# smdogroup/eigd

Measured on AMD Instinct MI355X. Metric: adjoint_mode_derivatives_per_sec, higher is better.
Workload: dtype f64

## Files before the change

eigd_amd/_ffi.py:

```python

import ctypes as C
import os

import numpy as np

_HERE = os.path.dirname(os.path.abspath(__file__))
LIB_PATH = os.environ.get("EIGD_LIB") or os.path.join(_HERE, "lib", "libeigd_hip.so")

EIGD_E_INVALID, EIGD_E_HIP, EIGD_E_NOTSPD, EIGD_E_INTERNAL = -1, -2, -3, -4


class EigdHipError(RuntimeError):
    """HIP runtime / device failure inside libeigd_hip.so."""


class NotPositiveDefiniteError(np.linalg.LinAlgError):
    """The shifted matrix handed to SpLuOperator is not positive definite."""


_lib = None

c_int, c_i64, c_dbl, c_sz, c_vp = C.c_int, C.c_int64, C.c_double, C.c_size_t, C.c_void_p
P = C.POINTER

_SIGNATURES = {
    "eigd_version": [],
    "eigd_device_count": [P(c_int)],
    "eigd_ctx_create": [c_int, P(c_vp)],
    "eigd_ctx_fork": [c_vp, P(c_vp)],
    "eigd_ctx_destroy": [c_vp],
    "eigd_ctx_make_current": [c_vp],
    "eigd_sync": [c_vp],
    "eigd_malloc": [c_vp, c_sz, P(c_vp)],
    "eigd_free": [c_vp, c_vp],
    "eigd_memset": [c_vp, c_vp, c_int, c_sz],
    "eigd_h2d": [c_vp, c_vp, c_vp, c_sz],
    "eigd_d2h": [c_vp, c_vp, c_vp, c_sz],
    "eigd_d2d": [c_vp, c_vp, c_vp, c_sz],
    "eigd_host_alloc": [c_sz, P(c_vp)],
    "eigd_host_free": [c_vp],
    "eigd_host_register": [c_vp, c_sz],
    "eigd_host_unregister": [c_vp],
    "eigd_mem_info": [c_vp, P(c_sz), P(c_sz)],
    "eigd_timer_start": [c_vp],
    "eigd_timer_stop_ms": [c_vp, P(c_dbl)],
    "eigd_csr_upload": [c_vp, c_int, c_i64, c_vp, c_vp, c_vp, P(c_vp)],
    "eigd_csr_upload_rect": [c_vp, c_int, c_int, c_i64, c_vp, c_vp, c_vp, P(c_vp)],
    "eigd_csr_update_values": [c_vp, c_vp],
    "eigd_csr_transpose_pattern": [c_int, c_int, c_vp, c_vp, c_vp, c_vp, c_vp],
    "eigd_csr_transpose": [c_vp, P(c_vp)],
    "eigd_csr_transpose_refresh": [c_vp, c_vp],
    "eigd_mat_free": [c_vp],
    "eigd_spmm": [c_vp, c_vp, c_int, c_vp, c_int, c_int, c_dbl, c_dbl],
    "eigd_spmm_on": [c_vp, c_vp, c_vp, c_int, c_vp, c_int, c_int, c_dbl, c_dbl],
    "eigd_ccsr_upload": [c_vp, c_int, c_i64, c_vp, c_vp, c_vp, P(c_vp)],
    "eigd_ccsr_update_values_dev": [c_vp, c_vp],
    "eigd_ccsr_conjugate_transpose": [c_vp, P(c_vp)],
    "eigd_ccsr_conjugate_transpose_refresh": [c_vp, c_vp],
    "eigd_ccsr_spmm_on": [c_vp, c_vp, c_vp, c_int, c_vp, c_int, c_int, c_dbl, c_dbl],
    "eigd_expand_values": [c_vp, c_i64, c_i64, c_vp, c_vp, c_vp],
    "eigd_symbolic_create": [c_int, c_vp, c_vp, c_int, c_int, P(c_vp)],
    "eigd_symbolic_create_geom": [c_int, c_vp, c_vp, c_int, c_int, c_int, c_vp, P(c_vp)],
    "eigd_symbolic_free": [c_vp],
    "eigd_symbolic_sizes": [c_vp, c_vp, c_int],
    "eigd_symbolic_sweep_plan": [c_vp, c_int, c_int, c_int, c_vp, c_vp, c_int, P(c_int)],
    "eigd_symbolic_get_i32": [c_vp, C.c_char_p, c_vp, c_i64],
    "eigd_symbolic_get_i64": [c_vp, C.c_char_p, c_vp, c_i64],
    "eigd_factor_create": [c_vp, c_vp, c_vp, P(c_vp)],
    "eigd_factor_create_lu": [c_vp, c_vp, c_vp, P(c_vp)],
    "eigd_factor_refactor": [c_vp, c_vp],
# ... 113 lines not shown
```

eigd_amd/csrc/sparse.hip:

```cpp
#include <algorithm>
#include <cstdint>
#include <vector>

#include "common.h"

struct eigd_mat {
  eigd_ctx* ctx = nullptr;
  int n = 0;
  int ncols = 0;
  int64_t nnz = 0;
  int32_t* indptr = nullptr;
  int32_t* indices = nullptr;
  double* data = nullptr;
  int32_t* rowblocks = nullptr;
  int nblocks = 0;
  int ntiles = 0, umax = 0;
  int tnz_cap = 0;
  int32_t* tile_ptr = nullptr;
  int32_t* ucols = nullptr;
  uint16_t* lidx = nullptr;
  int32_t* tperm = nullptr;
  double* cdata = nullptr;
};

namespace eigd {

constexpr int kTileRows = 32;
constexpr int kTileLds = 40 * 1024;
constexpr int kTileNnz = 1024;
constexpr int kNnzTile = 2048;
constexpr int kMaxRowsTile = 256;


__device__ __forceinline__ int xcd_remap(int b, int nblocks_padded) {
  const int per = nblocks_padded >> 3;
  return (b & 7) * per + (b >> 3);
}

__global__ __launch_bounds__(kThreads) void spmv_stream_kernel(const int32_t* __restrict__ rowblocks, int nblocks,
                                                              int nblocks_padded,
                                                              const int32_t* __restrict__ indptr,
                                                              const int32_t* __restrict__ indices,
                                                              const double* __restrict__ vals,
                                                              const double* __restrict__ x, double* __restrict__ y,
                                                              double alpha, double beta) {
  __shared__ double prod[kNnzTile];
  __shared__ double red[kThreads];
  const int b = xcd_remap(blockIdx.x, nblocks_padded);
  if (b >= nblocks) return;
  const int tid = threadIdx.x;
// ... 62 lines not shown
  const int r = blockIdx.x * RP + threadIdx.x / KP;
  if (r >= n || c >= k) return;
  const int a = indptr[r], z = indptr[r + 1];
  double s = 0.0;
  int e = a;
  for (; e + 8 <= z; e += 8) {
    int col[8];
    double v[8], x[8];
#pragma unroll
    for (int q = 0; q < 8; ++q) {
      col[q] = indices[e + q];
      v[q] = vals[e + q];
    }
#pragma unroll
    for (int q = 0; q < 8; ++q) x[q] = X[static_cast<int64_t>(col[q]) * ldx + c];
#pragma unroll
    for (int q = 0; q < 8; ++q) s = __dadd_rn(s, __dmul_rn(v[q], x[q]));
  }
  for (; e < z; ++e) s = __dadd_rn(s, __dmul_rn(vals[e], X[static_cast<int64_t>(indices[e]) * ldx + c]));
  double* yp = Y + static_cast<int64_t>(r) * ldy + c;
  *yp = (beta == 0.0) ? alpha * s : alpha * s + beta * (*yp);
}

template <int KP, int LANES = 8>
struct SpmmTile {
  static constexpr int CPL = (KP >= LANES) ? KP / LANES : 1;
  static constexpr int LPR = KP / CPL;
  static constexpr int LD = (CPL >= 2) ? KP + 4 : KP + 1;
};

template <int KP, int LANES, bool DOTS = false>
__global__ __launch_bounds__(kThreads) void spmm_tiled_kernel(int n, int k, int ntiles, int tiles_per_xcd,
                                                             const int32_t* __restrict__ tile_ptr,
                                                             const int32_t* __restrict__ ucols,
                                                             const int32_t* __restrict__ indptr,
                                                             const uint16_t* __restrict__ lidx,
                                                             const double* __restrict__ vals,
                                                             const double* __restrict__ X, int ldx,
                                                             double* __restrict__ Y, int ldy, double alpha, double beta,
                                                             int umax, int tnz_cap,
                                                             const double* __restrict__ R = nullptr, int ldr = 0,
                                                             double* __restrict__ dots = nullptr) {
  extern __shared__ __align__(16) double Xs[];
  constexpr int RP = kThreads / KP;
  constexpr int CPL = SpmmTile<KP, LANES>::CPL, LPR = SpmmTile<KP, LANES>::LPR, LD = SpmmTile<KP, LANES>::LD;
  constexpr int RPP = kThreads / LPR;
  constexpr int NR = (kTileRows + RPP - 1) / RPP;
  double* const Vs = Xs + static_cast<size_t>(umax) * LD;
  uint16_t* const Ls = reinterpret_cast<uint16_t*>(Vs + tnz_cap);
  const int tile = (blockIdx.x & 7) * tiles_per_xcd + (blockIdx.x >> 3);
  if (tile >= ntiles) return;
  const int c = threadIdx.x % KP, rr = threadIdx.x / KP;
  const int pl = threadIdx.x % LPR, prow = threadIdx.x / LPR;
  const int u0 = tile_ptr[tile], nu = tile_ptr[tile + 1] - u0;
  const int rend = min(n, (tile + 1) * kTileRows);
  const int e0 = indptr[tile * kTileRows], tnz = indptr[rend] - e0;
  const bool staged = tnz <= tnz_cap;
  constexpr int NQ = kTileNnz / kThreads;
  int ra[NR], rz[NR];
#pragma unroll
  for (int i = 0; i < NR; ++i) {
    const int r = tile * kTileRows + prow + i * RPP;
    ra[i] = (r < rend) ? indptr[r] - e0 : 0;
    rz[i] = (r < rend) ? indptr[r + 1] - e0 : 0;
  }
  double sv[NQ];
  uint16_t sl[NQ];
#pragma unroll
  for (int q = 0; q < NQ; ++q) {
    const int e = threadIdx.x + q * kThreads;
    const bool ok = staged && e < tnz;
    sv[q] = ok ? vals[e0 + e] : 0.0;
    sl[q] = ok ? lidx[e0 + e] : uint16_t(0);
  }
  [[maybe_unused]] double xo[CPL], ro[CPL];
  if constexpr (DOTS) {
    const int r = tile * kTileRows + prow;
#pragma unroll
    for (int t = 0; t < CPL; ++t) {
      const bool ok = r < rend && CPL * pl + t < k;
      xo[t] = ok ? X[static_cast<int64_t>(r) * ldx + CPL * pl + t] : 0.0;
      ro[t] = ok ? R[static_cast<int64_t>(r) * ldr + CPL * pl + t] : 0.0;
    }
  }
  constexpr int SU = 16;
  for (int j0 = 0; j0 < nu; j0 += SU * RP) {
    int col[SU];
    double x[SU];
#pragma unroll
    for (int q = 0; q < SU; ++q) {
      const int j = j0 + q * RP + rr;
      col[q] = (j < nu) ? ucols[u0 + j] : -1;
    }
#pragma unroll
    for (int q = 0; q < SU; ++q) x[q] = (col[q] >= 0 && c < k) ? X[static_cast<int64_t>(col[q]) * ldx + c] : 0.0;
#pragma unroll
    for (int q = 0; q < SU; ++q) {
      const int j = j0 + q * RP + rr;
      if (j < nu) Xs[j * LD + c] = x[q];
    }
  }
  if (staged) {
#pragma unroll
// ... 40 lines not shown
#pragma unroll
        for (int w = 0; w < kThreads / 64; ++w) v += dred[(w * 2 + q) * KP + c2];
        dots[static_cast<int64_t>(tile) * 2 * k + threadIdx.x] = v;
      }
    }
  };
  auto store_row = [&](int r, const double (&s)[CPL]) {
    double* yp = Y + static_cast<int64_t>(r) * ldy + cb;
#pragma unroll
    for (int t = 0; t < CPL; ++t)
      if (cb + t < k) {
        const double yv = (beta == 0.0) ? alpha * s[t] : alpha * s[t] + beta * yp[t];
        yp[t] = yv;
        if constexpr (DOTS) {
          dzr[t] += xo[t] * ro[t];
          dzy[t] += xo[t] * yv;
        }
      }
  };
  const bool active = cb < k;
  if (active && staged) {
#pragma unroll
    for (int i = 0; i < NR; ++i) {
      const int r = tile * kTileRows + prow + i * RPP;
      if (r >= rend) break;
      const int a = ra[i], z = rz[i];
      double s[CPL];
#pragma unroll
      for (int t = 0; t < CPL; ++t) s[t] = 0.0;
      int e = a;
      for (; e + 8 <= z; e += 8) {
        int li[8];
        double v[8], x[8][CPL];
#pragma unroll
        for (int q = 0; q < 8; ++q) {
          li[q] = Ls[e + q];
          v[q] = Vs[e + q];
        }
#pragma unroll
        for (int q = 0; q < 8; ++q) {
          const double* xp = Xs + li[q] * LD + cb;
          if constexpr (CPL >= 2) {
            const double2* xp2 = reinterpret_cast<const double2*>(xp);
#pragma unroll
            for (int t = 0; t < CPL / 2; ++t) {
              const double2 w = xp2[t];
              x[q][2 * t] = w.x;
              x[q][2 * t + 1] = w.y;
            }
          } else {
            x[q][0] = xp[0];
          }
        }
#pragma unroll
        for (int q = 0; q < 8; ++q)
#pragma unroll
          for (int t = 0; t < CPL; ++t) s[t] = __dadd_rn(s[t], __dmul_rn(v[q], x[q][t]));
      }
      for (; e < z; ++e) {
        const double v = Vs[e];
        const double* xp = Xs + Ls[e] * LD + cb;
#pragma unroll
        for (int t = 0; t < CPL; ++t) s[t] = __dadd_rn(s[t], __dmul_rn(v, xp[t]));
      }
      store_row(r, s);
    }
  } else if (active) {
  for (int r = tile * kTileRows + prow; r < rend; r += RPP) {
    const int a = indptr[r], z = indptr[r + 1];
    double s[CPL];
#pragma unroll
    for (int t = 0; t < CPL; ++t) s[t] = 0.0;
    for (int e = a; e < z; ++e) {
      const double v = vals[e];
      const double* xp = Xs + lidx[e] * LD + cb;
#pragma unroll
      for (int t = 0; t < CPL; ++t) s[t] = __dadd_rn(s[t], __dmul_rn(v, xp[t]));
    }
    store_row(r, s);
  }
  }
  finish_dots();
}

__global__ __launch_bounds__(kThreads) void tile_dots_reduce_kernel(const double* __restrict__ dots, int ntiles, int nout,
                                                                   double* __restrict__ out) {
  __shared__ double red[kThreads];
  const int per = kThreads / nout;
  const int o = threadIdx.x % nout, sub = threadIdx.x / nout;
  double v = 0.0;
  if (sub < per)
// ... 88 lines not shown
        si = __dadd_rn(si, pi[q]);
      }
      store(r, sr, si);
    }
  } else {
    double sr = 0.0, si = 0.0;
    for (int ea = e0; ea < e1; ea += kNnzTile) {
      const int ez = min(e1, ea + kNnzTile);
      stage(ea, ez);
      __syncthreads();
      if (tid == 0)
        for (int q = 0; q < ez - ea; ++q) {
          sr = __dadd_rn(sr, pr[q]);
          si = __dadd_rn(si, pi[q]);
        }
      __syncthreads();
    }
    if (tid == 0) store(r0, sr, si);
  }
}

template <bool STAGED>
__global__ __launch_bounds__(kThreads) void cspmm_tiled_kernel(int n, int kb, int kp_log2, int ntiles, int tiles_per_xcd,
                                                              const int32_t* __restrict__ tile_ptr,
                                                              const int32_t* __restrict__ ucols,
                                                              const int32_t* __restrict__ indptr,
                                                              const int32_t* __restrict__ indices,
                                                              const uint16_t* __restrict__ lidx,
                                                              const cdbl2* __restrict__ vals,
                                                              const double* __restrict__ X, int ldx, int imx,
                                                              double* __restrict__ Y, int ldy, int imy, double alpha,
                                                              double beta) {
  extern __shared__ __align__(16) double Xs[];
  const int tile = (blockIdx.x & 7) * tiles_per_xcd + (blockIdx.x >> 3);
  if (tile >= ntiles) return;
  const int kp = 1 << kp_log2;
  const int c = threadIdx.x & (kp - 1), rr = threadIdx.x >> kp_log2;
  const int rpp = kThreads >> kp_log2;
  const int ld = 2 * kp + 1;
  const int rbeg = tile * kTileRows, rend = min(n, rbeg + kTileRows);
  if constexpr (STAGED) {
    const int u0 = tile_ptr[tile], nu = tile_ptr[tile + 1] - u0;
    constexpr int SU = 8;
    for (int j0 = 0; j0 < nu; j0 += SU * rpp) {
      int col[SU];
      double xr[SU], xi[SU];
#pragma unroll
      for (int q = 0; q < SU; ++q) {
        const int j = j0 + q * rpp + rr;
        col[q] = (j < nu) ? ucols[u0 + j] : -1;
      }
#pragma unroll
      for (int q = 0; q < SU; ++q) {
        const bool ok = col[q] >= 0 && c < kb;
        const double* xp = X + static_cast<int64_t>(ok ? col[q] : 0) * ldx + (ok ? c : 0);
        xr[q] = ok ? xp[0] : 0.0;
        xi[q] = ok ? xp[imx] : 0.0;
      }
#pragma unroll
      for (int q = 0; q < SU; ++q) {
        const int j = j0 + q * rpp + rr;
        if (j < nu) {
          Xs[j * ld + c] = xr[q];
          Xs[j * ld + kp + c] = xi[q];
        }
      }
    }
    __syncthreads();
  }
  if (c >= kb) return;
  for (int r = rbeg + rr; r < rend; r += rpp) {
    const int a = indptr[r], z = indptr[r + 1];
    CAcc s;
    int e = a;
    for (; e + 4 <= z; e += 4) {
      cdbl2 v[4];
      double xr[4], xi[4];
#pragma unroll
      for (int q = 0; q < 4; ++q) {
        v[q] = vals[e + q];
        if constexpr (STAGED) {
          const double* xp = Xs + static_cast<int>(lidx[e + q]) * ld + c;
          xr[q] = xp[0];
          xi[q] = xp[kp];
        } else {
          const double* xp = X + static_cast<int64_t>(indices[e + q]) * ldx + c;
          xr[q] = xp[0];
          xi[q] = xp[imx];
        }
      }
#pragma unroll
      for (int q = 0; q < 4; ++q) s.add(v[q][0], v[q][1], xr[q], xi[q]);
    }
    for (; e < z; ++e) {
// ... 3 lines not shown
        s.add(v[0], v[1], xp[0], xp[kp]);
      } else {
        const double* xp = X + static_cast<int64_t>(indices[e]) * ldx + c;
        s.add(v[0], v[1], xp[0], xp[imx]);
      }
    }
    double* yp = Y + static_cast<int64_t>(r) * ldy + c;
    yp[0] = (beta == 0.0) ? alpha * s.re : alpha * s.re + beta * yp[0];
    yp[imy] = (beta == 0.0) ? alpha * s.im : alpha * s.im + beta * yp[imy];
  }
}

__global__ __launch_bounds__(kThreads) void expand_values_kernel(int64_t nout, const int32_t* __restrict__ table,
                                                                const double* __restrict__ src, double* __restrict__ dst) {
  const int64_t stride = static_cast<int64_t>(gridDim.x) * kThreads;
  for (int64_t q = static_cast<int64_t>(blockIdx.x) * kThreads + threadIdx.x; q < nout; q += stride) {
    const int32_t t = table[q];
    double v = 0.0;
    if (t >= 0) {
      v = src[2 * static_cast<int64_t>(t >> 2) + ((t >> 1) & 1)];
      if (t & 1) v = -v;
    }
    dst[q] = v;
  }
}

}

using namespace eigd;

extern "C" {

int eigd_csr_upload(eigd_ctx* ctx, int n, int64_t nnz, const int32_t* hindptr, const int32_t* hindices,
                    const double* hdata, eigd_mat** out) {
  return eigd_csr_upload_rect(ctx, n, n, nnz, hindptr, hindices, hdata, out);
}

int eigd_csr_upload_rect(eigd_ctx* ctx, int n, int ncols, int64_t nnz, const int32_t* hindptr, const int32_t* hindices,
                         const double* hdata, eigd_mat** out) {
  EIGD_REQUIRE(ctx && hindptr && hindices && hdata && out, "null argument");
  EIGD_REQUIRE(n > 0 && ncols > 0 && nnz >= 0 && nnz < (int64_t(1) << 31), "bad matrix size %d x %d nnz=%lld", n, ncols,
               (long long)nnz);
  EIGD_REQUIRE(hindptr[0] == 0 && hindptr[n] == nnz, "indptr does not match nnz");
  for (int i = 0; i < n; ++i) EIGD_REQUIRE(hindptr[i + 1] >= hindptr[i], "indptr not monotone at row %d", i);
  for (int64_t e = 0; e < nnz; ++e)
    EIGD_REQUIRE(hindices[e] >= 0 && hindices[e] < ncols, "column index out of range at entry %lld", (long long)e);
  *out = nullptr;
  std::vector<int32_t> rb;
  rb.push_back(0);
  {
    int r = 0;
    while (r < n) {
      int start = r;
      int64_t cnt = 0;
      while (r < n && (r - start) < kMaxRowsTile) {
        int64_t len = hindptr[r + 1] - hindptr[r];
        if (cnt + len > kNnzTile - 2) break;
        cnt += len;
        ++r;
      }
      if (r == start) ++r;
      rb.push_back(r);
    }
  }
  const int ntiles = (n + kTileRows - 1) / kTileRows;
  std::vector<int32_t> tile_ptr(static_cast<size_t>(ntiles) + 1, 0), ucols;
  std::vector<uint16_t> lidx(static_cast<size_t>(nnz) + 8, 0);
  int umax = 0;
  int64_t tnz_max = 0;
  bool tiles_ok = true;
  {
    std::vector<int32_t> cols, stamp(static_cast<size_t>(ncols), -1), pos(static_cast<size_t>(ncols), 0);
    ucols.reserve(static_cast<size_t>(nnz) / 4 + 16);
    for (int t = 0; t < ntiles && tiles_ok; ++t) {
      const int r0 = t * kTileRows, r1 = std::min(n, r0 + kTileRows);
      cols.clear();
      for (int64_t e = hindptr[r0]; e < hindptr[r1]; ++e) {
        const int32_t cidx = hindices[e];
        if (stamp[cidx] != t) {
          stamp[cidx] = t;
          cols.push_back(cidx);
        }
      }
      std::sort(cols.begin(), cols.end());
      if (cols.size() > 65535) tiles_ok = false;
      umax = std::max<int>(umax, static_cast<int>(cols.size()));
      tnz_max = std::max<int64_t>(tnz_max, hindptr[r1] - hindptr[r0]);
      for (size_t q = 0; q < cols.size(); ++q) pos[cols[q]] = static_cast<int32_t>(q);
      for (int64_t e = hindptr[r0]; e < hindptr[r1]; ++e) lidx[e] = static_cast<uint16_t>(pos[hindices[e]]);
      ucols.insert(ucols.end(), cols.begin(), cols.end());
      tile_ptr[t + 1] = static_cast<int32_t>(ucols.size());
    }
  }
  EIGD_HIP(hipSetDevice(ctx->device));
  eigd_mat* A = new eigd_mat();
  A->ctx = ctx;
  A->n = n;
  A->ncols = ncols;
  A->nnz = nnz;
  A->nblocks = static_cast<int>(rb.size()) - 1;
  if (tiles_ok) {
    A->ntiles = ntiles;
    A->umax = umax;
    A->tnz_cap = static_cast<int>(std::min<int64_t>(kTileNnz, (tnz_max + 7) & ~int64_t(7)));
    hipError_t t1 = hipMalloc(reinterpret_cast<void**>(&A->tile_ptr), sizeof(int32_t) * tile_ptr.size());
    hipError_t t2 = hipMalloc(reinterpret_cast<void**>(&A->ucols), sizeof(int32_t) * std::max<size_t>(ucols.size(), 1));
    hipError_t t3 = hipMalloc(reinterpret_cast<void**>(&A->lidx), sizeof(uint16_t) * lidx.size());
    if (t1 != hipSuccess || t2 != hipSuccess || t3 != hipSuccess) {
      eigd_mat_free(A);
      set_error("hipMalloc failed for the SpMM tiles (n=%d nnz=%lld)", n, (long long)nnz);
      return EIGD_E_HIP;
    }
    EIGD_HIP(hipMemcpy(A->tile_ptr, tile_ptr.data(), sizeof(int32_t) * tile_ptr.size(), hipMemcpyHostToDevice));
    if (!ucols.empty()) EIGD_HIP(hipMemcpy(A->ucols, ucols.data(), sizeof(int32_t) * ucols.size(), hipMemcpyHostToDevice));
    EIGD_HIP(hipMemcpy(A->lidx, lidx.data(), sizeof(uint16_t) * lidx.size(), hipMemcpyHostToDevice));
  }
  hipError_t e1 = hipMalloc(reinterpret_cast<void**>(&A->indptr), sizeof(int32_t) * (n + 1));
  hipError_t e2 = hipMalloc(reinterpret_cast<void**>(&A->indices), sizeof(int32_t) * (nnz + 4));
  hipError_t e3 = hipMalloc(reinterpret_cast<void**>(&A->data), sizeof(double) * (nnz + 4));
  hipError_t e4 = hipMalloc(reinterpret_cast<void**>(&A->rowblocks), sizeof(int32_t) * rb.size());
  if (e1 != hipSuccess || e2 != hipSuccess || e3 != hipSuccess || e4 != hipSuccess) {
    eigd_mat_free(A);
    set_error("hipMalloc failed for CSR matrix (n=%d nnz=%lld)", n, (long long)nnz);
    return EIGD_E_HIP;
  }
  EIGD_HIP(hipMemcpy(A->indptr, hindptr, sizeof(int32_t) * (n + 1), hipMemcpyHostToDevice));
  if (nnz > 0) {
    EIGD_HIP(hipMemcpy(A->indices, hindices, sizeof(int32_t) * nnz, hipMemcpyHostToDevice));
    EIGD_HIP(hipMemcpy(A->data, hdata, sizeof(double) * nnz, hipMemcpyHostToDevice));
  }
  EIGD_HIP(hipMemcpy(A->rowblocks, rb.data(), sizeof(int32_t) * rb.size(), hipMemcpyHostToDevice));
  *out = A;
  return EIGD_OK;
}

int eigd_csr_update_values(eigd_mat* A, const double* hdata) {
  EIGD_REQUIRE(A && hdata, "null argument");
  EIGD_REQUIRE(!A->cdata, "a complex matrix: its values are updated on the device (eigd_ccsr_update_values_dev)");
  EIGD_HIP(hipStreamSynchronize(A->ctx->stream));
  if (A->nnz > 0) EIGD_HIP(hipMemcpy(A->data, hdata, sizeof(double) * A->nnz, hipMemcpyHostToDevice));
  return EIGD_OK;
}

int eigd_csr_update_values_dev(eigd_mat* A, const double* dvals) {
  EIGD_REQUIRE(A && dvals, "null argument");
  EIGD_REQUIRE(!A->cdata, "a complex matrix: use eigd_ccsr_update_values_dev");
  if (A->nnz > 0)
    EIGD_HIP(hipMemcpyAsync(A->data, dvals, sizeof(double) * A->nnz, hipMemcpyDeviceToDevice, A->ctx->stream));
  return EIGD_OK;
}

int eigd_csr_transpose_pattern(int n, int ncols, const int32_t* indptr, const int32_t* indices, int32_t* t_indptr,
                               int32_t* t_indices, int32_t* t_perm) {
  EIGD_REQUIRE(indptr && indices && t_indptr && t_indices && t_perm, "null argument");
  EIGD_REQUIRE(n >= 0 && ncols >= 0 && indptr[0] == 0, "bad matrix size %d x %d", n, ncols);
// ... 44 lines not shown
  if (nnz > 0) EIGD_HIP(hipMemcpy(At->tperm, perm.data(), sizeof(int32_t) * nnz, hipMemcpyHostToDevice));
  *out = At;
  return EIGD_OK;
}

int eigd_csr_transpose_refresh(eigd_mat* At, eigd_mat* A) {
  EIGD_REQUIRE(At && A, "null argument");
  EIGD_REQUIRE(At->tperm && At->nnz == A->nnz && At->n == A->ncols && At->ctx->device == A->ctx->device,
               "not a transposed companion of this matrix");
  if (A->nnz == 0) return EIGD_OK;
  const int nb = static_cast<int>(std::min<int64_t>((A->nnz + kThreads - 1) / kThreads, 65536));
  hipLaunchKernelGGL(gather_values_kernel, dim3(nb), dim3(kThreads), 0, A->ctx->stream, A->nnz, At->tperm, A->data, At->data);
  EIGD_LAUNCH_CHECK();
  return EIGD_OK;
}

int eigd_mat_free(eigd_mat* A) {
  if (!A) return EIGD_OK;
  if (A->ctx && A->ctx->stream) (void)hipStreamSynchronize(A->ctx->stream);
  if (A->indptr) (void)hipFree(A->indptr);
  if (A->indices) (void)hipFree(A->indices);
  if (A->data) (void)hipFree(A->data);
  if (A->rowblocks) (void)hipFree(A->rowblocks);
  if (A->tile_ptr) (void)hipFree(A->tile_ptr);
  if (A->ucols) (void)hipFree(A->ucols);
  if (A->lidx) (void)hipFree(A->lidx);
  if (A->tperm) (void)hipFree(A->tperm);
  if (A->cdata) (void)hipFree(A->cdata);
  delete A;
  return EIGD_OK;
}

int eigd_spmm(eigd_mat* A, const double* dX, int ldx, double* dY, int ldy, int k, double alpha, double beta) {
  EIGD_REQUIRE(A, "null argument");
  return eigd_spmm_on(A->ctx, A, dX, ldx, dY, ldy, k, alpha, beta);
}

int eigd_spmm_on(eigd_ctx* ctx, eigd_mat* A, const double* dX, int ldx, double* dY, int ldy, int k, double alpha,
                 double beta) {
  EIGD_REQUIRE(ctx && A && dX && dY, "null argument");
  EIGD_REQUIRE(ctx->device == A->ctx->device, "context and matrix live on different devices");
  EIGD_REQUIRE(k >= 1 && ldx >= k && ldy >= k, "bad block shape k=%d ldx=%d ldy=%d", k, ldx, ldy);
  EIGD_REQUIRE(dX != dY, "spmm cannot run in place");
  EIGD_REQUIRE(!A->cdata, "a complex matrix: use eigd_ccsr_spmm_on");
  hipStream_t st = ctx->stream;
  if (k == 1 && ldx == 1 && ldy == 1) {
// ... 2 lines not shown
                       A->indices, A->data, dX, dY, alpha, beta);
    EIGD_LAUNCH_CHECK();
    return EIGD_OK;
  }
  auto tile_fits = [&](int kpv) {
    const int cplv = (kpv >= 8) ? kpv / 8 : 1;
    return A->ntiles > 0 && sizeof(double) * static_cast<size_t>(A->umax) * (cplv >= 2 ? kpv + 4 : kpv + 1) <= static_cast<size_t>(kTileLds);
  };
  const int chunk = (k > 32 && !tile_fits(64) && tile_fits(32)) ? 32 : kMaxK;
  for (int c0 = 0; c0 < k; c0 += chunk) {
    const int kb = std::min(chunk, k - c0);
    const int kp = std::max(2, next_pow2(kb));
    const int rp = kThreads / kp;
    const dim3 grid((A->n + rp - 1) / rp);
    const int cpl = (kp >= 8) ? kp / 8 : 1;
    const size_t tile_lds = sizeof(double) * static_cast<size_t>(A->umax) * (cpl >= 2 ? kp + 4 : kp + 1);
    const size_t tile_lds_all = tile_lds + static_cast<size_t>(A->tnz_cap) * (sizeof(double) + sizeof(uint16_t));
    if (A->ntiles > 0 && tile_lds <= static_cast<size_t>(kTileLds)) {
      const int per_xcd = (A->ntiles + 7) / 8;
      const dim3 tgrid(per_xcd * 8);
#define EIGD_SPMM_TILED(KP)                                                                                            \
  case KP:                                                                                                             \
    hipLaunchKernelGGL((spmm_tiled_kernel<KP, 8>), tgrid, dim3(kThreads), tile_lds_all, st, A->n, kb, A->ntiles,       \
                       per_xcd, A->tile_ptr, A->ucols, A->indptr, A->lidx, A->data, dX + c0, ldx, dY + c0, ldy,        \
                       alpha, beta, A->umax, A->tnz_cap);                                                              \
    break;
      switch (kp) {
        EIGD_SPMM_TILED(2)
        EIGD_SPMM_TILED(4)
        EIGD_SPMM_TILED(8)
        EIGD_SPMM_TILED(16)
        EIGD_SPMM_TILED(32)
        EIGD_SPMM_TILED(64)
        default:
          set_error("internal: unexpected kp=%d", kp);
          return EIGD_E_INTERNAL;
      }
#undef EIGD_SPMM_TILED
      EIGD_LAUNCH_CHECK();
      continue;
    }
#define EIGD_SPMM_CASE(KP)                                                                                          \
  case KP:                                                                                                          \
    hipLaunchKernelGGL(spmm_rows_kernel<KP>, grid, dim3(kThreads), 0, st, A->n, kb, A->indptr, A->indices, A->data, \
                       dX + c0, ldx, dY + c0, ldy, alpha, beta);                                                    \
    break;
    switch (kp) {
// ... 21 lines not shown
  EIGD_REQUIRE(dZ != dY, "spmm cannot run in place");
  EIGD_REQUIRE(!A->cdata, "a complex matrix has no conjugate-gradient product");
  const int kp = std::max(2, next_pow2(k));
  const int cpl = (kp >= 8) ? kp / 8 : 1;
  const size_t tile_lds = sizeof(double) * static_cast<size_t>(A->umax) * (cpl >= 2 ? kp + 4 : kp + 1);
  const bool fused = kp >= 8 && kp <= 32 && A->ntiles > 0 && tile_lds <= static_cast<size_t>(kTileLds);
  if (!fused) {
    int rc = eigd_spmm_on(ctx, A, dZ, ldz, dY, ldy, k, 1.0, 0.0);
    if (rc) return rc;
    return eigd_cg_coefficients(ctx, A->n, k, dZ, ldz, dR, ldr, dY, ldy, dNorm2, dState, step, first, dLog);
  }
  const int groups = std::min(A->ntiles, 1024);
  int rc = ctx->ensure_scratch(sizeof(double) * (static_cast<size_t>(A->ntiles) + groups) * 2 * k);
  if (rc) return rc;
  double* gsum = ctx->scratch;
  double* dots = ctx->scratch + static_cast<size_t>(groups) * 2 * k;
  const size_t tile_lds_all = tile_lds + static_cast<size_t>(A->tnz_cap) * (sizeof(double) + sizeof(uint16_t));
  const int per_xcd = (A->ntiles + 7) / 8;
  const dim3 tgrid(per_xcd * 8);
  hipStream_t st = ctx->stream;
#define EIGD_SPMM_DOTS(KP)                                                                                             \
  case KP:                                                                                                             \
    hipLaunchKernelGGL((spmm_tiled_kernel<KP, 8, true>), tgrid, dim3(kThreads), tile_lds_all, st, A->n, k, A->ntiles,  \
                       per_xcd, A->tile_ptr, A->ucols, A->indptr, A->lidx, A->data, dZ, ldz, dY, ldy, 1.0, 0.0,        \
                       A->umax, A->tnz_cap, dR, ldr, dots);                                                            \
    break;
  switch (kp) {
    EIGD_SPMM_DOTS(8)
    EIGD_SPMM_DOTS(16)
    EIGD_SPMM_DOTS(32)
    default:
      set_error("internal: unexpected kp=%d", kp);
      return EIGD_E_INTERNAL;
  }
#undef EIGD_SPMM_DOTS
  EIGD_LAUNCH_CHECK();
  hipLaunchKernelGGL(tile_dots_reduce_kernel, dim3(groups), dim3(kThreads), 0, st, dots, A->ntiles, 2 * k, gsum);
  EIGD_LAUNCH_CHECK();
  return cg_coefficients_from_partials(ctx, gsum, groups, k, dNorm2, dState, step, first, dLog);
}

namespace {
constexpr size_t kCTileLds = 64 * 1024;

int launch_expand(hipStream_t st, int64_t nout, const int32_t* table, const double* src, double* dst) {
  if (nout == 0) return EIGD_OK;
  const int nb = static_cast<int>(std::min<int64_t>((nout + kThreads - 1) / kThreads, 65536));
// ... 88 lines not shown
}

int eigd_ccsr_spmm_on(eigd_ctx* ctx, eigd_mat* A, const double* dX, int ldx, double* dY, int ldy, int k, double alpha,
                      double beta) {
  EIGD_REQUIRE(ctx && A && dX && dY, "null argument");
  EIGD_REQUIRE(A->cdata, "not a complex matrix");
  EIGD_REQUIRE(ctx->device == A->ctx->device, "context and matrix live on different devices");
  EIGD_REQUIRE(k >= 1 && ldx >= 2 * k && ldy >= 2 * k, "bad block shape k=%d ldx=%d ldy=%d", k, ldx, ldy);
  EIGD_REQUIRE(dX != dY, "spmm cannot run in place");
  hipStream_t st = ctx->stream;
  const cdbl2* vals = reinterpret_cast<const cdbl2*>(A->cdata);
  if (k == 1) {
    const int nbp = (A->nblocks + 7) & ~7;
    hipLaunchKernelGGL(cspmv_stream_kernel, dim3(nbp), dim3(kThreads), 0, st, A->rowblocks, A->nblocks, nbp, A->indptr,
                       A->indices, vals, dX, ldx, 1, dY, ldy, 1, alpha, beta);
    EIGD_LAUNCH_CHECK();
    return EIGD_OK;
  }
  auto lds_of = [&](int kp) { return sizeof(double) * static_cast<size_t>(A->umax) * (2 * kp + 1); };
  int chunk = 32;
  while (chunk > 1 && (A->ntiles == 0 || lds_of(chunk) > kCTileLds)) chunk >>= 1;
  const bool staged = A->ntiles > 0 && lds_of(chunk) <= kCTileLds;
  if (!staged) chunk = 32;
  const int ntiles = (A->n + kTileRows - 1) / kTileRows;
  const int per_xcd = (ntiles + 7) / 8;
  const dim3 tgrid(per_xcd * 8);
  for (int c0 = 0; c0 < k; c0 += chunk) {
    const int kb = std::min(chunk, k - c0);
    const int kp = next_pow2(kb);
    int lg = 0;
    while ((1 << lg) < kp) ++lg;
    if (staged)
      hipLaunchKernelGGL(cspmm_tiled_kernel<true>, tgrid, dim3(kThreads), lds_of(kp), st, A->n, kb, lg, ntiles, per_xcd,
                         A->tile_ptr, A->ucols, A->indptr, A->indices, A->lidx, vals, dX + c0, ldx, k, dY + c0, ldy, k,
                         alpha, beta);
    else
      hipLaunchKernelGGL(cspmm_tiled_kernel<false>, tgrid, dim3(kThreads), 0, st, A->n, kb, lg, ntiles, per_xcd,
                         A->tile_ptr, A->ucols, A->indptr, A->indices, A->lidx, vals, dX + c0, ldx, k, dY + c0, ldy, k,
                         alpha, beta);
    EIGD_LAUNCH_CHECK();
  }
  return EIGD_OK;
}

}
```

eigd_amd/device.py:

```python

import contextlib
import ctypes as C

import numpy as np

from . import _ffi
from ._ffi import c_vp, call, hptr

_default_ctx = None


class Context:

    def __init__(self, device=0, _parent=None):
        h = c_vp()
        if _parent is None:
            call("eigd_ctx_create", int(device), C.byref(h))
        else:
            call("eigd_ctx_fork", _parent.h, C.byref(h))
        self.h = h
        self.device = int(device)
        self.parent = _parent

    def fork(self, index=0):
# ... 746 lines not shown
        for blk, a, b in self.pieces(j0, j0 + X.k):
            blk.copy_from(X.cols(a, b))

    def to_host(self, m):
        out = np.empty((self.n, m))
        for blk, a, b in self.pieces(0, m):
            out[:, a:b] = blk.get()
        return out

    def from_host(self, V):
        V = np.asarray(V, dtype=np.float64)
        for blk, a, b in self.pieces(0, V.shape[1]):
            blk.set(np.ascontiguousarray(V[:, a:b]))

    def as_stack(self, m):
        st = DeviceStack(self.ctx, m, self.n, 1)
        for blk, a, b in self.pieces(0, m):
            for q in range(b - a):
                st[a + q].copy_from(blk.cols(q, q + 1))
        return st

    def swap(self, other):
        self.buf, other.buf = other.buf, self.buf


class CSRMatrix:

    def __init__(self, ctx, A):
        from scipy import sparse

        A = sparse.csr_matrix(A)
        if A.dtype != np.float64:
            A = A.astype(np.float64)
        self.ctx = ctx
        self.shape = A.shape
        self.n, self.ncols = A.shape
        self.nnz = int(A.nnz)
        ip = np.ascontiguousarray(A.indptr, dtype=np.int32)
        ix = np.ascontiguousarray(A.indices, dtype=np.int32)
        dv = np.ascontiguousarray(A.data, dtype=np.float64)
        h = c_vp()
        call("eigd_csr_upload_rect", ctx.h, self.n, self.ncols, self.nnz, hptr(ip), hptr(ix), hptr(dv), C.byref(h))
        self.h = h
        self._transposed = None

    @classmethod
# ... 704 lines not shown
```

include/eigd_hip.h:

```cpp
#ifndef EIGD_HIP_H
#define EIGD_HIP_H

#include <stddef.h>
#include <stdint.h>

#ifdef __cplusplus
extern "C" {
#endif

#define EIGD_OK 0
#define EIGD_E_INVALID (-1)
#define EIGD_E_HIP (-2)
#define EIGD_E_NOTSPD (-3)
#define EIGD_E_INTERNAL (-4)

typedef struct eigd_ctx eigd_ctx;
typedef struct eigd_mat eigd_mat;
typedef struct eigd_symbolic eigd_symbolic;
typedef struct eigd_factor eigd_factor;
typedef struct eigd_lane eigd_lane;

const char* eigd_last_error(void);
int eigd_version(void);

// ... 1 lines not shown
int eigd_ctx_create(int device, eigd_ctx** out);
int eigd_ctx_fork(eigd_ctx* parent, eigd_ctx** out);
int eigd_ctx_destroy(eigd_ctx* ctx);
int eigd_ctx_make_current(eigd_ctx* ctx);
int eigd_sync(eigd_ctx* ctx);
int eigd_malloc(eigd_ctx* ctx, size_t bytes, void** dptr);
int eigd_free(eigd_ctx* ctx, void* dptr);
int eigd_memset(eigd_ctx* ctx, void* dptr, int value, size_t bytes);
int eigd_h2d(eigd_ctx* ctx, void* dptr, const void* hsrc, size_t bytes);
int eigd_d2h(eigd_ctx* ctx, void* hdst, const void* dptr, size_t bytes);
int eigd_d2d(eigd_ctx* ctx, void* ddst, const void* dsrc, size_t bytes);
int eigd_host_alloc(size_t bytes, void** hptr);
int eigd_host_free(void* hptr);
int eigd_host_register(void* hptr, size_t bytes);
int eigd_host_unregister(void* hptr);
int eigd_mem_info(eigd_ctx* ctx, size_t* free_bytes, size_t* total_bytes);
int eigd_timer_start(eigd_ctx* ctx);
int eigd_timer_stop_ms(eigd_ctx* ctx, double* ms);

int eigd_csr_upload(eigd_ctx* ctx, int n, int64_t nnz, const int32_t* hindptr, const int32_t* hindices,
                    const double* hdata, eigd_mat** out);
int eigd_csr_upload_rect(eigd_ctx* ctx, int n, int ncols, int64_t nnz, const int32_t* hindptr, const int32_t* hindices,
                         const double* hdata, eigd_mat** out);
int eigd_csr_update_values(eigd_mat* A, const double* hdata);
int eigd_csr_update_values_dev(eigd_mat* A, const double* dvals);
int eigd_csr_transpose_pattern(int n, int ncols, const int32_t* indptr, const int32_t* indices, int32_t* t_indptr,
                               int32_t* t_indices, int32_t* t_perm);
int eigd_csr_transpose(eigd_mat* A, eigd_mat** At);
int eigd_csr_transpose_refresh(eigd_mat* At, eigd_mat* A);
int eigd_mat_free(eigd_mat* A);
int eigd_spmm(eigd_mat* A, const double* dX, int ldx, double* dY, int ldy, int k, double alpha, double beta);
int eigd_spmm_on(eigd_ctx* ctx, eigd_mat* A, const double* dX, int ldx, double* dY, int ldy, int k, double alpha,
                 double beta);

int eigd_ccsr_upload(eigd_ctx* ctx, int n, int64_t nnz, const int32_t* hindptr, const int32_t* hindices,
                     const double* hdata, eigd_mat** out);
int eigd_ccsr_update_values_dev(eigd_mat* A, const double* dvals);
int eigd_ccsr_conjugate_transpose(eigd_mat* A, eigd_mat** Ah);
int eigd_ccsr_conjugate_transpose_refresh(eigd_mat* Ah, eigd_mat* A);
int eigd_ccsr_spmm_on(eigd_ctx* ctx, eigd_mat* A, const double* dX, int ldx, double* dY, int ldy, int k, double alpha,
                      double beta);
int eigd_expand_values(eigd_ctx* ctx, int64_t nout, int64_t nsrc, const int32_t* dtable, const double* dsrc,
                       double* ddst);

int eigd_symbolic_create(int n, const int32_t* hindptr, const int32_t* hindices, int leaf_size, int panel_width,
                         eigd_symbolic** out);
// ... 120 lines not shown
```

Baseline: 680.1.

## Build SpMM tiles from up to four row runs chosen by connectivity

Replaces fixed 32-row SpMM tiles with tiles made of up to four contiguous row runs. Runs are picked greedily by following column indices to untaken rows, and the run count (1, 2 or 4) that minimises total unique columns per tile is kept. The aim is to shrink the staged set of X rows in LDS and cut gather traffic. In exchange, the kernels pay extra per-row and per-nonzero index remapping through the run records, and matrix upload does more host-side preprocessing.

New measurement: 686.9 (median of 6 runs). Within noise of the previous version (+1.0%).

```diff
diff --git a/eigd_amd/_ffi.py b/eigd_amd/_ffi.py
--- a/eigd_amd/_ffi.py
+++ b/eigd_amd/_ffi.py
@@ -46,6 +46,7 @@
     "eigd_timer_stop_ms": [c_vp, P(c_dbl)],
     "eigd_csr_upload": [c_vp, c_int, c_i64, c_vp, c_vp, c_vp, P(c_vp)],
     "eigd_csr_upload_rect": [c_vp, c_int, c_int, c_i64, c_vp, c_vp, c_vp, P(c_vp)],
+    "eigd_spmm_tiling": [c_int, c_int, c_vp, c_vp, c_int, c_vp, c_int, c_vp],
     "eigd_csr_update_values": [c_vp, c_vp],
     "eigd_csr_transpose_pattern": [c_int, c_int, c_vp, c_vp, c_vp, c_vp, c_vp],
     "eigd_csr_transpose": [c_vp, P(c_vp)],
diff --git a/eigd_amd/csrc/sparse.hip b/eigd_amd/csrc/sparse.hip
--- a/eigd_amd/csrc/sparse.hip
+++ b/eigd_amd/csrc/sparse.hip
@@ -1,5 +1,6 @@
 #include <algorithm>
 #include <cstdint>
+#include <cstdlib>
 #include <vector>
 
 #include "common.h"
@@ -16,6 +17,8 @@
   int nblocks = 0;
   int ntiles = 0, umax = 0;
   int tnz_cap = 0;
+  int tile_runs = 0;
+  int32_t* tile_rec = nullptr;
   int32_t* tile_ptr = nullptr;
   int32_t* ucols = nullptr;
   uint16_t* lidx = nullptr;
@@ -26,6 +29,8 @@
 namespace eigd {
 
 constexpr int kTileRows = 32;
+constexpr int kTileRuns = 4;
+constexpr int kTileRec = 16;
 constexpr int kTileLds = 40 * 1024;
 constexpr int kTileNnz = 1024;
 constexpr int kNnzTile = 2048;
@@ -134,6 +139,53 @@
   *yp = (beta == 0.0) ? alpha * s : alpha * s + beta * (*yp);
 }
 
+struct TileRec {
+  int row[kTileRuns], nz[kTileRuns], rp[kTileRuns], ep[kTileRuns];
+  __device__ __forceinline__ explicit TileRec(const int32_t* __restrict__ w) {
+#pragma unroll
+    for (int q = 0; q < kTileRuns; ++q) {
+      row[q] = w[q];
+      nz[q] = w[kTileRuns + q];
+      rp[q] = w[2 * kTileRuns + q];
+      ep[q] = w[3 * kTileRuns + q];
+    }
+  }
+  __device__ __forceinline__ TileRec(int tile, int n) {
+    const int r0 = tile * kTileRows, m = min(n, r0 + kTileRows) - r0;
+#pragma unroll
+    for (int q = 0; q < kTileRuns; ++q) {
+      row[q] = r0;
+      nz[q] = 0;
+      rp[q] = m;
+      ep[q] = 0;
+    }
+  }
+  __device__ __forceinline__ int rows() const { return rp[kTileRuns - 1]; }
+  __device__ __forceinline__ int nnz() const { return ep[kTileRuns - 1]; }
+  __device__ __forceinline__ int row_of(int p, int& shift) const {
+    int r = row[0] + p;
+    shift = -nz[0];
+#pragma unroll
+    for (int q = 1; q < kTileRuns; ++q)
+      if (p >= rp[q - 1]) {
+        r = row[q] + (p - rp[q - 1]);
+        shift = ep[q - 1] - nz[q];
+      }
+    return r;
+  }
+  __device__ __forceinline__ int row_of(int p) const {
+    int shift;
+    return row_of(p, shift);
+  }
+  __device__ __forceinline__ int nz_of(int e) const {
+    int g = nz[0] + e;
+#pragma unroll
+    for (int q = 1; q < kTileRuns; ++q)
+      if (e >= ep[q - 1]) g = nz[q] + (e - ep[q - 1]);
+    return g;
+  }
+};
+
 template <int KP, int LANES = 8>
 struct SpmmTile {
   static constexpr int CPL = (KP >= LANES) ? KP / LANES : 1;
@@ -143,6 +195,7 @@
 
 template <int KP, int LANES, bool DOTS = false>
 __global__ __launch_bounds__(kThreads) void spmm_tiled_kernel(int n, int k, int ntiles, int tiles_per_xcd,
+                                                             const int32_t* __restrict__ tile_rec,
                                                              const int32_t* __restrict__ tile_ptr,
                                                              const int32_t* __restrict__ ucols,
                                                              const int32_t* __restrict__ indptr,
@@ -165,16 +218,16 @@
   const int c = threadIdx.x % KP, rr = threadIdx.x / KP;
   const int pl = threadIdx.x % LPR, prow = threadIdx.x / LPR;
   const int u0 = tile_ptr[tile], nu = tile_ptr[tile + 1] - u0;
-  const int rend = min(n, (tile + 1) * kTileRows);
-  const int e0 = indptr[tile * kTileRows], tnz = indptr[rend] - e0;
+  const TileRec tr(tile_rec + static_cast<int64_t>(tile) * kTileRec);
+  const int trows = tr.rows(), tnz = tr.nnz();
   const bool staged = tnz <= tnz_cap;
   constexpr int NQ = kTileNnz / kThreads;
-  int ra[NR], rz[NR];
+  int rw[NR], ra[NR], rz[NR], rs[NR];
 #pragma unroll
   for (int i = 0; i < NR; ++i) {
-    const int r = tile * kTileRows + prow + i * RPP;
-    ra[i] = (r < rend) ? indptr[r] - e0 : 0;
-    rz[i] = (r < rend) ? indptr[r + 1] - e0 : 0;
+    rw[i] = tr.row_of(min(prow + i * RPP, trows - 1), rs[i]);
+    ra[i] = indptr[rw[i]];
+    rz[i] = indptr[rw[i] + 1];
   }
   double sv[NQ];
   uint16_t sl[NQ];
@@ -182,15 +235,16 @@
   for (int q = 0; q < NQ; ++q) {
     const int e = threadIdx.x + q * kThreads;
     const bool ok = staged && e < tnz;
-    sv[q] = ok ? vals[e0 + e] : 0.0;
-    sl[q] = ok ? lidx[e0 + e] : uint16_t(0);
+    const int g = tr.nz_of(e);
+    sv[q] = ok ? vals[g] : 0.0;
+    sl[q] = ok ? lidx[g] : uint16_t(0);
   }
   [[maybe_unused]] double xo[CPL], ro[CPL];
   if constexpr (DOTS) {
-    const int r = tile * kTileRows + prow;
+    const int r = rw[0];
 #pragma unroll
     for (int t = 0; t < CPL; ++t) {
-      const bool ok = r < rend && CPL * pl + t < k;
+      const bool ok = prow < trows && CPL * pl + t < k;
       xo[t] = ok ? X[static_cast<int64_t>(r) * ldx + CPL * pl + t] : 0.0;
       ro[t] = ok ? R[static_cast<int64_t>(r) * ldr + CPL * pl + t] : 0.0;
     }
@@ -277,9 +331,9 @@
   if (active && staged) {
 #pragma unroll
     for (int i = 0; i < NR; ++i) {
-      const int r = tile * kTileRows + prow + i * RPP;
-      if (r >= rend) break;
-      const int a = ra[i], z = rz[i];
+      if (prow + i * RPP >= trows) break;
+      const int r = rw[i];
+      const int a = ra[i] + rs[i], z = rz[i] + rs[i];
       double s[CPL];
 #pragma unroll
       for (int t = 0; t < CPL; ++t) s[t] = 0.0;
@@ -321,7 +375,8 @@
       store_row(r, s);
     }
   } else if (active) {
-  for (int r = tile * kTileRows + prow; r < rend; r += RPP) {
+  for (int p = prow; p < trows; p += RPP) {
+    const int r = tr.row_of(p);
     const int a = indptr[r], z = indptr[r + 1];
     double s[CPL];
 #pragma unroll
@@ -456,6 +511,7 @@
 
 template <bool STAGED>
 __global__ __launch_bounds__(kThreads) void cspmm_tiled_kernel(int n, int kb, int kp_log2, int ntiles, int tiles_per_xcd,
+                                                              const int32_t* __restrict__ tile_rec,
                                                               const int32_t* __restrict__ tile_ptr,
                                                               const int32_t* __restrict__ ucols,
                                                               const int32_t* __restrict__ indptr,
@@ -472,7 +528,8 @@
   const int c = threadIdx.x & (kp - 1), rr = threadIdx.x >> kp_log2;
   const int rpp = kThreads >> kp_log2;
   const int ld = 2 * kp + 1;
-  const int rbeg = tile * kTileRows, rend = min(n, rbeg + kTileRows);
+  const TileRec tr = (tile_rec != nullptr) ? TileRec(tile_rec + static_cast<int64_t>(tile) * kTileRec) : TileRec(tile, n);
+  const int trows = tr.rows();
   if constexpr (STAGED) {
     const int u0 = tile_ptr[tile], nu = tile_ptr[tile + 1] - u0;
     constexpr int SU = 8;
@@ -503,7 +560,8 @@
     __syncthreads();
   }
   if (c >= kb) return;
-  for (int r = rbeg + rr; r < rend; r += rpp) {
+  for (int p = rr; p < trows; p += rpp) {
+    const int r = tr.row_of(p);
     const int a = indptr[r], z = indptr[r + 1];
     CAcc s;
     int e = a;
@@ -553,6 +611,108 @@
       if (t & 1) v = -v;
     }
     dst[q] = v;
+  }
+}
+
+struct SpmmTiling {
+  int runs = 0;
+  std::vector<int32_t> rec;
+  std::vector<int32_t> tile_ptr;
+  std::vector<int32_t> ucols;
+  int umax = 0;
+  int64_t tnz_max = 0;
+  bool ok = true;
+  int ntiles() const { return static_cast<int>(tile_ptr.size()) - 1; }
+  int64_t sum_ucols() const { return static_cast<int64_t>(ucols.size()); }
+};
+
+static void build_tiling(int n, int ncols, const int32_t* indptr, const int32_t* indices, int runs, SpmmTiling& T) {
+  T = SpmmTiling();
+  T.runs = runs;
+  T.tile_ptr.push_back(0);
+  const int len_max = kTileRows / runs;
+  std::vector<uint8_t> taken(static_cast<size_t>(n), 0);
+  std::vector<int32_t> stamp(static_cast<size_t>(ncols), -1), cols;
+  int next = 0, tile = 0;
+  while (true) {
+    while (next < n && taken[next]) ++next;
+    if (next >= n) break;
+    int row[kTileRuns], len[kTileRuns], nr = 0, left = kTileRows, start = next;
+    while (true) {
+      int m = 0;
+      while (m < std::min(len_max, left) && start + m < n && !taken[start + m]) taken[start + m++] = 1;
+      if (nr > 0 && row[nr - 1] + len[nr - 1] == start) {
+        len[nr - 1] += m;
+      } else {
+        row[nr] = start;
+        len[nr] = m;
+        ++nr;
+      }
+      left -= m;
+      if (left == 0 || nr == runs) break;
+      const int end = start + m;
+      int cand = -1;
+      for (int32_t e = indptr[start]; e < indptr[start + 1]; ++e) {
+        const int32_t c = indices[e];
+        if (c >= end && c < n && !taken[c] && (cand < 0 || c < cand)) cand = c;
+      }
+      if (cand < 0 && end < n && !taken[end]) cand = end;
+      if (cand < 0) break;
+      start = cand;
+    }
+    int32_t w[kTileRec];
+    int rp = 0, ep = 0;
+    cols.clear();
+    for (int q = 0; q < kTileRuns; ++q) {
+      if (q < nr) {
+        w[q] = row[q];
+        w[kTileRuns + q] = indptr[row[q]];
+        rp += len[q];
+        ep += indptr[row[q] + len[q]] - indptr[row[q]];
+        for (int32_t e = indptr[row[q]]; e < indptr[row[q] + len[q]]; ++e) {
+          const int32_t c = indices[e];
+          if (stamp[c] != tile) {
+            stamp[c] = tile;
+            cols.push_back(c);
+          }
+        }
+      } else {
+        w[q] = row[nr - 1];
+        w[kTileRuns + q] = indptr[row[nr - 1]];
+      }
+      w[2 * kTileRuns + q] = rp;
+      w[3 * kTileRuns + q] = ep;
+    }
+    std::sort(cols.begin(), cols.end());
+    if (cols.size() > 65535) T.ok = false;
+    T.umax = std::max<int>(T.umax, static_cast<int>(cols.size()));
+    T.tnz_max = std::max<int64_t>(T.tnz_max, ep);
+    T.rec.insert(T.rec.end(), w, w + kTileRec);
+    T.ucols.insert(T.ucols.end(), cols.begin(), cols.end());
+    T.tile_ptr.push_back(static_cast<int32_t>(T.ucols.size()));
+    ++tile;
+  }
+}
+
+static int forced_runs(int runs) {
+  if (runs == 0) {
+    const char* e = std::getenv("EIGD_SPMM_RUNS");
+    if (e && *e) runs = std::atoi(e);
+  }
+  return (runs == 1 || runs == 2 || runs == 4) ? runs : 0;
+}
+
+static void choose_tiling(int n, int ncols, const int32_t* indptr, const int32_t* indices, int runs, SpmmTiling& best) {
+  runs = forced_runs(runs);
+  if (runs) {
+    build_tiling(n, ncols, indptr, indices, runs, best);
+    return;
+  }
+  build_tiling(n, ncols, indptr, indices, 1, best);
+  for (int r = 2; r <= kTileRuns; r *= 2) {
+    SpmmTiling T;
+    build_tiling(n, ncols, indptr, indices, r, T);
+    if (T.ok && (!best.ok || T.sum_ucols() < best.sum_ucols())) best = std::move(T);
   }
 }
 
@@ -594,33 +754,22 @@
       rb.push_back(r);
     }
   }
-  const int ntiles = (n + kTileRows - 1) / kTileRows;
-  std::vector<int32_t> tile_ptr(static_cast<size_t>(ntiles) + 1, 0), ucols;
+  SpmmTiling T;
+  choose_tiling(n, ncols, hindptr, hindices, 0, T);
+  const bool tiles_ok = T.ok;
+  const int ntiles = T.ntiles(), umax = T.umax;
+  const int64_t tnz_max = T.tnz_max;
+  const std::vector<int32_t>&tile_ptr = T.tile_ptr, &ucols = T.ucols;
   std::vector<uint16_t> lidx(static_cast<size_t>(nnz) + 8, 0);
-  int umax = 0;
-  int64_t tnz_max = 0;
-  bool tiles_ok = true;
-  {
-    std::vector<int32_t> cols, stamp(static_cast<size_t>(ncols), -1), pos(static_cast<size_t>(ncols), 0);
-    ucols.reserve(static_cast<size_t>(nnz) / 4 + 16);
-    for (int t = 0; t < ntiles && tiles_ok; ++t) {
-      const int r0 = t * kTileRows, r1 = std::min(n, r0 + kTileRows);
-      cols.clear();
-      for (int64_t e = hindptr[r0]; e < hindptr[r1]; ++e) {
-        const int32_t cidx = hindices[e];
-        if (stamp[cidx] != t) {
-          stamp[cidx] = t;
-          cols.push_back(cidx);
-        }
-      }
-      std::sort(cols.begin(), cols.end());
-      if (cols.size() > 65535) tiles_ok = false;
-      umax = std::max<int>(umax, static_cast<int>(cols.size()));
-      tnz_max = std::max<int64_t>(tnz_max, hindptr[r1] - hindptr[r0]);
-      for (size_t q = 0; q < cols.size(); ++q) pos[cols[q]] = static_cast<int32_t>(q);
-      for (int64_t e = hindptr[r0]; e < hindptr[r1]; ++e) lidx[e] = static_cast<uint16_t>(pos[hindices[e]]);
-      ucols.insert(ucols.end(), cols.begin(), cols.end());
-      tile_ptr[t + 1] = static_cast<int32_t>(ucols.size());
+  if (tiles_ok) {
+    std::vector<int32_t> pos(static_cast<size_t>(ncols), 0);
+    for (int t = 0; t < ntiles; ++t) {
+      for (int32_t q = tile_ptr[t]; q < tile_ptr[t + 1]; ++q) pos[ucols[q]] = q - tile_ptr[t];
+      const int32_t* w = T.rec.data() + static_cast<size_t>(t) * kTileRec;
+      for (int q = 0; q < kTileRuns; ++q) {
+        const int32_t e0 = w[kTileRuns + q], cnt = w[3 * kTileRuns + q] - (q ? w[3 * kTileRuns + q - 1] : 0);
+        for (int32_t e = e0; e < e0 + cnt; ++e) lidx[e] = static_cast<uint16_t>(pos[hindices[e]]);
+      }
     }
   }
   EIGD_HIP(hipSetDevice(ctx->device));
@@ -632,16 +781,19 @@
   A->nblocks = static_cast<int>(rb.size()) - 1;
   if (tiles_ok) {
     A->ntiles = ntiles;
+    A->tile_runs = T.runs;
     A->umax = umax;
     A->tnz_cap = static_cast<int>(std::min<int64_t>(kTileNnz, (tnz_max + 7) & ~int64_t(7)));
     hipError_t t1 = hipMalloc(reinterpret_cast<void**>(&A->tile_ptr), sizeof(int32_t) * tile_ptr.size());
     hipError_t t2 = hipMalloc(reinterpret_cast<void**>(&A->ucols), sizeof(int32_t) * std::max<size_t>(ucols.size(), 1));
     hipError_t t3 = hipMalloc(reinterpret_cast<void**>(&A->lidx), sizeof(uint16_t) * lidx.size());
-    if (t1 != hipSuccess || t2 != hipSuccess || t3 != hipSuccess) {
+    hipError_t t4 = hipMalloc(reinterpret_cast<void**>(&A->tile_rec), sizeof(int32_t) * T.rec.size());
+    if (t1 != hipSuccess || t2 != hipSuccess || t3 != hipSuccess || t4 != hipSuccess) {
       eigd_mat_free(A);
       set_error("hipMalloc failed for the SpMM tiles (n=%d nnz=%lld)", n, (long long)nnz);
       return EIGD_E_HIP;
     }
+    EIGD_HIP(hipMemcpy(A->tile_rec, T.rec.data(), sizeof(int32_t) * T.rec.size(), hipMemcpyHostToDevice));
     EIGD_HIP(hipMemcpy(A->tile_ptr, tile_ptr.data(), sizeof(int32_t) * tile_ptr.size(), hipMemcpyHostToDevice));
     if (!ucols.empty()) EIGD_HIP(hipMemcpy(A->ucols, ucols.data(), sizeof(int32_t) * ucols.size(), hipMemcpyHostToDevice));
     EIGD_HIP(hipMemcpy(A->lidx, lidx.data(), sizeof(uint16_t) * lidx.size(), hipMemcpyHostToDevice));
@@ -662,6 +814,28 @@
   }
   EIGD_HIP(hipMemcpy(A->rowblocks, rb.data(), sizeof(int32_t) * rb.size(), hipMemcpyHostToDevice));
   *out = A;
+  return EIGD_OK;
+}
+
+int eigd_spmm_tiling(int n, int ncols, const int32_t* indptr, const int32_t* indices, int runs, int32_t* rec, int cap,
+                     int* info) {
+  EIGD_REQUIRE(indptr && indices && info, "null argument");
+  EIGD_REQUIRE(n > 0 && ncols > 0 && indptr[0] == 0, "bad matrix size %d x %d", n, ncols);
+  EIGD_REQUIRE(runs == 0 || runs == 1 || runs == 2 || runs == 4, "runs = 0 (the library's choice), 1, 2 or 4, not %d", runs);
+  EIGD_REQUIRE(cap >= 0 && (cap == 0 || rec != nullptr), "bad capacity");
+  for (int i = 0; i < n; ++i) EIGD_REQUIRE(indptr[i + 1] >= indptr[i], "indptr not monotone at row %d", i);
+  for (int64_t e = 0; e < indptr[n]; ++e)
+    EIGD_REQUIRE(indices[e] >= 0 && indices[e] < ncols, "column index out of range at entry %lld", (long long)e);
+  SpmmTiling T;
+  choose_tiling(n, ncols, indptr, indices, runs, T);
+  info[0] = T.ntiles();
+  info[1] = T.runs;
+  info[2] = T.umax;
+  info[3] = T.ok ? 1 : 0;
+  info[4] = static_cast<int>(T.sum_ucols() & 0x7fffffff);
+  info[5] = static_cast<int>(T.sum_ucols() >> 31);
+  const int m = std::min(cap, T.ntiles());
+  std::copy(T.rec.begin(), T.rec.begin() + static_cast<size_t>(m) * kTileRec, rec);
   return EIGD_OK;
 }
 
@@ -752,6 +926,7 @@
   if (A->indices) (void)hipFree(A->indices);
   if (A->data) (void)hipFree(A->data);
   if (A->rowblocks) (void)hipFree(A->rowblocks);
+  if (A->tile_rec) (void)hipFree(A->tile_rec);
   if (A->tile_ptr) (void)hipFree(A->tile_ptr);
   if (A->ucols) (void)hipFree(A->ucols);
   if (A->lidx) (void)hipFree(A->lidx);
@@ -800,7 +975,7 @@
 #define EIGD_SPMM_TILED(KP)                                                                                            \
   case KP:                                                                                                             \
     hipLaunchKernelGGL((spmm_tiled_kernel<KP, 8>), tgrid, dim3(kThreads), tile_lds_all, st, A->n, kb, A->ntiles,       \
-                       per_xcd, A->tile_ptr, A->ucols, A->indptr, A->lidx, A->data, dX + c0, ldx, dY + c0, ldy,        \
+                       per_xcd, A->tile_rec, A->tile_ptr, A->ucols, A->indptr, A->lidx, A->data, dX + c0, ldx, dY + c0, ldy,        \
                        alpha, beta, A->umax, A->tnz_cap);                                                              \
     break;
       switch (kp) {
@@ -868,7 +1043,7 @@
 #define EIGD_SPMM_DOTS(KP)                                                                                             \
   case KP:                                                                                                             \
     hipLaunchKernelGGL((spmm_tiled_kernel<KP, 8, true>), tgrid, dim3(kThreads), tile_lds_all, st, A->n, k, A->ntiles,  \
-                       per_xcd, A->tile_ptr, A->ucols, A->indptr, A->lidx, A->data, dZ, ldz, dY, ldy, 1.0, 0.0,        \
+                       per_xcd, A->tile_rec, A->tile_ptr, A->ucols, A->indptr, A->lidx, A->data, dZ, ldz, dY, ldy, 1.0, 0.0,        \
                        A->umax, A->tnz_cap, dR, ldr, dots);                                                            \
     break;
   switch (kp) {
@@ -1003,7 +1178,7 @@
   while (chunk > 1 && (A->ntiles == 0 || lds_of(chunk) > kCTileLds)) chunk >>= 1;
   const bool staged = A->ntiles > 0 && lds_of(chunk) <= kCTileLds;
   if (!staged) chunk = 32;
-  const int ntiles = (A->n + kTileRows - 1) / kTileRows;
+  const int ntiles = A->ntiles > 0 ? A->ntiles : (A->n + kTileRows - 1) / kTileRows;
   const int per_xcd = (ntiles + 7) / 8;
   const dim3 tgrid(per_xcd * 8);
   for (int c0 = 0; c0 < k; c0 += chunk) {
@@ -1013,11 +1188,11 @@
     while ((1 << lg) < kp) ++lg;
     if (staged)
       hipLaunchKernelGGL(cspmm_tiled_kernel<true>, tgrid, dim3(kThreads), lds_of(kp), st, A->n, kb, lg, ntiles, per_xcd,
-                         A->tile_ptr, A->ucols, A->indptr, A->indices, A->lidx, vals, dX + c0, ldx, k, dY + c0, ldy, k,
+                         A->tile_rec, A->tile_ptr, A->ucols, A->indptr, A->indices, A->lidx, vals, dX + c0, ldx, k, dY + c0, ldy, k,
                          alpha, beta);
     else
       hipLaunchKernelGGL(cspmm_tiled_kernel<false>, tgrid, dim3(kThreads), 0, st, A->n, kb, lg, ntiles, per_xcd,
-                         A->tile_ptr, A->ucols, A->indptr, A->indices, A->lidx, vals, dX + c0, ldx, k, dY + c0, ldy, k,
+                         A->tile_rec, A->tile_ptr, A->ucols, A->indptr, A->indices, A->lidx, vals, dX + c0, ldx, k, dY + c0, ldy, k,
                          alpha, beta);
     EIGD_LAUNCH_CHECK();
   }
diff --git a/eigd_amd/device.py b/eigd_amd/device.py
--- a/eigd_amd/device.py
+++ b/eigd_amd/device.py
@@ -792,6 +792,23 @@
 
     def swap(self, other):
         self.buf, other.buf = other.buf, self.buf
+
+
+def spmm_tiling(A, runs=0):
+    from scipy import sparse
+
+    A = sparse.csr_matrix(A)
+    ip = np.ascontiguousarray(A.indptr, dtype=np.int32)
+    ix = np.ascontiguousarray(A.indices, dtype=np.int32)
+    info = np.zeros(6, dtype=np.int32)
+    call("eigd_spmm_tiling", A.shape[0], A.shape[1], hptr(ip), hptr(ix), int(runs), None, 0, hptr(info))
+    rec = np.zeros((max(int(info[0]), 1), 16), dtype=np.int32)
+    call("eigd_spmm_tiling", A.shape[0], A.shape[1], hptr(ip), hptr(ix), int(runs), hptr(rec), int(info[0]), hptr(info))
+    rec = rec[:int(info[0])]
+    rows = np.diff(rec[:, 8:12], axis=1, prepend=0)
+    tiles = [[(int(t[q]), int(m[q]), int(t[4 + q])) for q in range(4) if m[q] > 0] for t, m in zip(rec, rows)]
+    return {"runs": int(info[1]), "tiles": tiles, "sum_ucols": int(info[4]) + (int(info[5]) << 31), "umax": int(info[2]),
+            "tiled": bool(info[3])}
 
 
 class CSRMatrix:
diff --git a/include/eigd_hip.h b/include/eigd_hip.h
--- a/include/eigd_hip.h
+++ b/include/eigd_hip.h
@@ -47,6 +47,8 @@
                     const double* hdata, eigd_mat** out);
 int eigd_csr_upload_rect(eigd_ctx* ctx, int n, int ncols, int64_t nnz, const int32_t* hindptr, const int32_t* hindices,
                          const double* hdata, eigd_mat** out);
+int eigd_spmm_tiling(int n, int ncols, const int32_t* indptr, const int32_t* indices, int runs, int32_t* rec, int cap,
+                     int* info);
 int eigd_csr_update_values(eigd_mat* A, const double* hdata);
 int eigd_csr_update_values_dev(eigd_mat* A, const double* dvals);
 int eigd_csr_transpose_pattern(int n, int ncols, const int32_t* indptr, const int32_t* indices, int32_t* t_indptr,
```
